# Loveof1ife7/mini-3d-gaussian-splatting

Measured on AMD Instinct MI355X. Metric: rendered Mpix/s fwd+bwd @1080p, 1M Gaussians; PSNR vs ref; 1/2/4/8-GPU scaling, higher is better.
Workload: dtype f32; 1 GPU; C3: 1,000,000 synthetic Gaussians (SURVEY 8d), 1920x1080, 16x16 tiles, render fwd+bwd + Adam step; preset=C3, gaussians=1000000, width=1920, height=1080, parallelism=dp1 (one view per GPU)

## Files before the change

mini-3d-gaussian-splatting_amd/csrc/gs_bin.hip:

```cpp
#include <hip/hip_runtime.h>
#include <stdint.h>

#include "gsplat_mi355x.h"
#include "gs_internal.h"
#include "gs_device.h"

namespace {

#ifndef GS_RANGES_X4
#define GS_RANGES_X4 1
#endif
constexpr int kBinChunk = kBlock * 4;

__device__ __forceinline__ uint2 *sorted_rects(uint32_t *partials, int nb) {
  return reinterpret_cast<uint2 *>(partials + ((5 * nb + 3) & ~3));
}

__global__ __launch_bounds__(kBlock) void k_bin_partials(gs_bin_args a, uint32_t *partials, int nb) {
  __shared__ uint32_t s_tmp3[3][kBlock / kWave];
  const long long base = (long long)blockIdx.x * kBinChunk;
  constexpr int kR = kBinChunk / kBlock;
  uint32_t gi[kR];
  uint2 rc_own[kR];
#pragma unroll
  for (int i = 0; i < kR; ++i) {
    const long long k = base + i * kBlock + threadIdx.x;
    const long long kc = k < a.n ? k : a.n - 1;
    gi[i] = a.sorted_ids[kc];
    rc_own[i] = reinterpret_cast<const uint2 *>(a.rects)[kc];
  }
  uint32_t sum = 0, nvis = 0;
  uint2 rc_d[kR];
  uint32_t vis_o[kR];
#pragma unroll
  for (int i = 0; i < kR; ++i) {
    const long long k = base + i * kBlock + threadIdx.x;
    rc_d[i] = reinterpret_cast<const uint2 *>(a.rects)[gi[i]];
    vis_o[i] = a.vis[k < a.n ? k : a.n - 1];
  }
#pragma unroll
  for (int i = 0; i < kR; ++i) {
    const long long k = base + i * kBlock + threadIdx.x;
    if (k < a.n) {
      sum += rect_touches((int)(rc_d[i].x & 0xFFFFu), (int)(rc_d[i].x >> 16), (int)(rc_d[i].y & 0xFFFFu),
                          (int)(rc_d[i].y >> 16));
      nvis += vis_o[i] ? 1u : 0u;
    }
  }
  uint32_t cnt[kR];
#pragma unroll
  for (int i = 0; i < kR; ++i) {
    const long long g = base + i * kBlock + threadIdx.x;
    cnt[i] = g < a.n ? rect_touches((int)(rc_own[i].x & 0xFFFFu), (int)(rc_own[i].x >> 16),
                                    (int)(rc_own[i].y & 0xFFFFu), (int)(rc_own[i].y >> 16))
                     : 0u;
  }
  uint3 t3;
  const uint3 e3 = block_exscan3(make_uint3(sum, nvis, cnt[0]), s_tmp3, &t3);
  if (threadIdx.x == 0) {
    partials[blockIdx.x] = t3.x;
    partials[nb + blockIdx.x] = t3.y;
  }
  uint2 *srect = sorted_rects(partials, nb);
#pragma unroll
  for (int i = 0; i < kR; ++i) {
    const long long k = base + i * kBlock + threadIdx.x;
    if (k < a.n) srect[k] = rc_d[i];
  }
  static_assert(kR == 4, "the slot prefix scans assume four rounds per binning block");
  uint3 u3;
  const uint3 f3 = block_exscan3(make_uint3(cnt[1], cnt[2], cnt[3]), s_tmp3, &u3);
  const uint32_t ex[kR] = {e3.z, f3.x, f3.y, f3.z};
  const uint32_t tt[kR] = {t3.z, u3.x, u3.y, u3.z};
  uint32_t carry = 0;
#pragma unroll
  for (int i = 0; i < kR; ++i) {
    const long long g = base + i * kBlock + threadIdx.x;
    if (g < a.n) a.pair_offset[g] = carry + ex[i];
    carry += tt[i];
  }
  if (threadIdx.x == 0) partials[2 * nb + blockIdx.x] = carry;
  constexpr int kPB = kBinChunk / kBlock;
  if (threadIdx.x < kPB) {
    const int pb = blockIdx.x * kPB + threadIdx.x, npb = (a.n + kBlock - 1) / kBlock;
    const bool ok = pb < npb;
    uint32_t mn = ok ? a.key_minmax[2 * pb] : 0xFFFFFFFFu, mx = ok ? a.key_minmax[2 * pb + 1] : 0u;
#pragma unroll
    for (int d = 1; d < kPB; d <<= 1) {
      mn = min(mn, (uint32_t)__shfl_xor((int)mn, d, 64));
      mx = max(mx, (uint32_t)__shfl_xor((int)mx, d, 64));
    }
    if (threadIdx.x == 0) {
      partials[3 * nb + blockIdx.x] = mn;
      partials[4 * nb + blockIdx.x] = mx;
    }
  }
}

__device__ __forceinline__ bool window_held(uint32_t key_base, int key_bits, uint32_t zmin, uint32_t zmax) {
  if (key_bits <= 0 || key_bits >= 32 || zmin > zmax) return true;
  const uint64_t full = (1ull << key_bits) - 1ull;
  const uint64_t lim = key_bits >= 9 ? min(full, 255ull << (key_bits - 8)) : full;
  return zmin >= key_base && (uint64_t)(zmax - key_base) < lim;
}

__global__ __launch_bounds__(kBlock) void k_bin_scan_partials(gs_bin_args a, uint32_t *partials, int nb) {
  uint32_t *const counters = a.counters, *const host_counters = a.host_counters;
  __shared__ uint32_t s_tmp3[3][kBlock / kWave];
  __shared__ uint32_t s_mm[2][kBlock / kWave];
  uint32_t mn = 0xFFFFFFFFu, mx = 0u;
  uint32_t carry = 0, vis = 0, slots = 0;
  auto ld = [&](int i, uint32_t *v) {
    const int ci = i < nb ? i : nb - 1;
    v[0] = partials[ci];
    v[1] = partials[nb + ci];
    v[2] = partials[2 * nb + ci];
    v[3] = partials[3 * nb + ci];
    v[4] = partials[4 * nb + ci];
  };
  uint32_t vn[5];
  ld((int)threadIdx.x, vn);
  for (int c = 0; c < nb; c += kBlock) {
    const int i = c + threadIdx.x;
    const uint32_t v0 = i < nb ? vn[0] : 0u, v1 = i < nb ? vn[1] : 0u, v2 = i < nb ? vn[2] : 0u;
    mn = min(mn, vn[3]);
    mx = max(mx, vn[4]);
    ld(i + kBlock, vn);
    uint3 t3;
    const uint3 e = block_exscan3(make_uint3(v0, v1, v2), s_tmp3, &t3);
    if (i < nb) {
      partials[i] = carry + e.x;
      partials[2 * nb + i] = slots + e.z;
    }
    carry += t3.x;
    vis += t3.y;
    slots += t3.z;
  }
#pragma unroll
  for (int d = 32; d >= 1; d >>= 1) {
    mn = min(mn, (uint32_t)__shfl_xor((int)mn, d, 64));
    mx = max(mx, (uint32_t)__shfl_xor((int)mx, d, 64));
  }
  if ((threadIdx.x & (kWave - 1)) == 0) {
    s_mm[0][threadIdx.x >> 6] = mn;
    s_mm[1][threadIdx.x >> 6] = mx;
  }
  __syncthreads();
  if (threadIdx.x == 0) {
#pragma unroll
    for (int w = 0; w < kBlock / kWave; ++w) {
      mn = min(mn, s_mm[0][w]);
      mx = max(mx, s_mm[1][w]);
    }
    uint32_t status = 0u;
    if ((long long)carry > a.capacity) status |= GS_FRAME_NEED_CAPACITY;
    if (!window_held(a.key_base, a.key_bits, mn, mx)) status |= GS_FRAME_WINDOW_MISS;
    if (vis == 0u) status |= GS_FRAME_EMPTY;
    counters[0] = vis;
    counters[1] = carry;
    counters[2] = mn;
    counters[3] = mx;
    counters[4] = status;
    counters[5] = status ? 0u : carry;
    uint32_t seq = a.host_seq;
    if (a.frame_seq) {
      seq = *a.frame_seq + 1u;
      *a.frame_seq = seq;
    }
    uint32_t sticky = status;
    bool first_fail = status != 0u;
    if (a.step_flags) {
      const uint32_t old = atomicOr(a.step_flags, status);
      sticky = old | status;
      first_fail = old == 0u && status != 0u;
    }
    if (host_counters) {
      host_counters[0] = vis;
      host_counters[1] = carry;
      host_counters[2] = mn;
      host_counters[3] = mx;
      host_counters[5] = status;
      host_counters[6] = sticky;
      if (first_fail) host_counters[7] = seq;
      __threadfence_system();
      host_counters[4] = seq;
      __threadfence_system();
    }
  }
}

constexpr uint32_t kWaveFillRun = 32;
template <typename Fill>
__device__ __forceinline__ void wave_fill_runs(bool wide, uint32_t lo, uint32_t hi, uint32_t value, Fill fill) {
  unsigned long long m = __ballot(wide);
  if (!m) return;
  const unsigned long long act = __ballot(1);
  const uint32_t lane = threadIdx.x & 63u;
  const uint32_t nact = (uint32_t)__popcll(act), rank = (uint32_t)__popcll(act & ((1ull << lane) - 1ull));
  while (m) {
    const int l = __ffsll(m) - 1;
    m &= m - 1;
    const uint32_t rlo = (uint32_t)__shfl((int)lo, l, 64), rhi = (uint32_t)__shfl((int)hi, l, 64);
    const uint32_t v = (uint32_t)__shfl((int)value, l, 64);
    for (uint32_t o = rlo + rank; o < rhi; o += nact) fill(o, v);
  }
}

constexpr uint32_t kOwnerCap = kBlock * 64;
__global__ __launch_bounds__(kBlock) void k_bin_emit(gs_bin_args a, const uint32_t *partials) {
  __shared__ uint32_t s_off[kBlock + 1];
  __shared__ uint32_t s_g[kBlock];
  __shared__ uint2 s_rect[kBlock];
  __shared__ uint32_t s_tmp[4];
  __shared__ uint32_t s_tmp3[3][kBlock / kWave];
  __shared__ uint8_t s_owner[kOwnerCap];
  const long long base = (long long)blockIdx.x * kBinChunk;
  if (a.device_counts && a.counters[4] != 0u) {
    for (int r = 0; r < kBinChunk / kBlock; ++r) {
      const long long g = base + r * kBlock + threadIdx.x;
      if (g < a.n) reinterpret_cast<uint2 *>(const_cast<uint32_t *>(a.rects))[g] = make_uint2(1u, 1u);
    }
    return;
  }
  const uint32_t T = a.counters[1];
  if ((long long)T > a.capacity) return;
  uint32_t out_base = partials[blockIdx.x];
  constexpr int kR = kBinChunk / kBlock;
  uint32_t gr[kR];
  uint2 rcr[kR];
  uint32_t offr[kR];
  const uint2 *srect = sorted_rects(const_cast<uint32_t *>(partials), (int)gridDim.x);
#pragma unroll
  for (int r = 0; r < kR; ++r) {
    const long long k = base + r * kBlock + threadIdx.x;
    const long long kc = k < a.n ? k : a.n - 1;
    gr[r] = a.sorted_ids[kc];
    rcr[r] = srect[kc];
    offr[r] = a.pair_offset[kc];
  }
  static_assert(kR == 4, "the emission's prefix scans assume four rounds per binning block");
  uint32_t cntr[kR];
#pragma unroll
  for (int r = 0; r < kR; ++r) {
    const long long k = base + r * kBlock + threadIdx.x;
    if (k < a.n) {
      cntr[r] = rect_touches((int)(rcr[r].x & 0xFFFFu), (int)(rcr[r].x >> 16), (int)(rcr[r].y & 0xFFFFu),
                             (int)(rcr[r].y >> 16));
    } else {
      cntr[r] = 0u;
      gr[r] = 0xFFFFFFFFu;
      rcr[r] = make_uint2(1u, 1u);
    }
  }
  uint3 ta;
  uint32_t tb;
  const uint3 ea = block_exscan3(make_uint3(cntr[0], cntr[1], cntr[2]), s_tmp3, &ta);
  const uint32_t eb = block_exscan(cntr[3], s_tmp, &tb);
  const uint32_t exr[kR] = {ea.x, ea.y, ea.z, eb}, totr[kR] = {ta.x, ta.y, ta.z, tb};
#pragma unroll
  for (int r = 0; r < kR; ++r) {
    const uint32_t g = gr[r], cnt = cntr[r], ex = exr[r], tot = totr[r];
    const uint2 rc = rcr[r];
    if (r) __syncthreads();
    s_off[threadIdx.x] = ex;
    s_g[threadIdx.x] = g;
    s_rect[threadIdx.x] = rc;
    if (threadIdx.x == 0) s_off[kBlock] = tot;
    for (uint32_t wb = 0; wb < tot; wb += kOwnerCap) {
      if (wb) __syncthreads();
      const uint32_t lo_c = ex > wb ? ex : wb, hi_c = min(ex + cnt, wb + kOwnerCap);
      const bool wide = hi_c > lo_c + kWaveFillRun;
      if (!wide)
        for (uint32_t o = lo_c; o < hi_c; ++o) s_owner[o - wb] = (uint8_t)threadIdx.x;
      wave_fill_runs(wide, lo_c - wb, hi_c - wb, threadIdx.x, [&](uint32_t o, uint32_t owner) {
        s_owner[o] = (uint8_t)owner;
      });
      __syncthreads();
      const uint32_t wend = min(tot, wb + kOwnerCap);
      for (uint32_t o = wb + threadIdx.x; o < wend; o += kBlock) {
        const int lo = s_owner[o - wb];
        const uint2 rr = s_rect[lo];
        const uint32_t tx0 = rr.x & 0xFFFFu, ty0 = rr.y & 0xFFFFu;
        const uint32_t wt = (rr.x >> 16) - tx0 + 1u;
        const uint32_t loc = o - s_off[lo];
        const uint32_t row = loc / wt;
        const uint32_t key = (ty0 + row) * (uint32_t)a.tiles_x + tx0 + (loc - row * wt);
        a.tile_keys[out_base + o] = key;
        a.pair_gauss[out_base + o] = s_g[lo];
      }
    }
    out_base += tot;
  }
  const uint32_t cbase = partials[2 * gridDim.x + blockIdx.x];
#pragma unroll
  for (int r = 0; r < kR; ++r) {
    const long long g = base + r * kBlock + threadIdx.x;
    if (g < a.n) {
      const uint32_t slot = cbase + offr[r];
      a.pair_offset[g] = slot;
      a.records[(size_t)g * GS_RECORD_FLOATS + 10] = __uint_as_float(slot);
    }
  }
}

__global__ __launch_bounds__(kBlock) void k_tile_ranges4(gs_range_args a) {
  const long long p0 = 4 * ((long long)blockIdx.x * kBlock + threadIdx.x);
  const long long T = live_items(a.num_pairs, a.num_pairs_dev);
  if (p0 > T) return;
  const int lane = threadIdx.x & 63;
  uint4 k = make_uint4(0u, 0u, 0u, 0u);
  if (p0 + 3 < T) {
    k = reinterpret_cast<const uint4 *>(a.sorted_keys)[p0 / 4];
  } else {
    if (p0 < T) k.x = a.sorted_keys[p0];
    if (p0 + 1 < T) k.y = a.sorted_keys[p0 + 1];
    if (p0 + 2 < T) k.z = a.sorted_keys[p0 + 2];
  }
  uint32_t before = (uint32_t)__shfl_up((int)k.w, 1, 64);
  if (lane == 0) before = p0 > 0 ? a.sorted_keys[p0 - 1] : 0u;
  if (a.slot_live) {
    if (p0 + 3 < T)
      reinterpret_cast<uint4 *>(a.slot_live)[p0 / 4] = make_uint4(0u, 0u, 0u, 0u);
    else
      for (long long q = p0; q < T; ++q) reinterpret_cast<uint32_t *>(a.slot_live)[q] = 0u;
  }
  const uint32_t kk[4] = {k.x, k.y, k.z, k.w};
#pragma unroll
  for (int i = 0; i < 4; ++i) {
    const long long p = p0 + i;
    const bool in = p <= T;
    const long long prev = !in ? 0 : (p > 0 ? (long long)(i ? kk[i - 1] : before) : -1);
    const long long cur = !in ? 0 : (p < T ? (long long)kk[i] : (long long)a.num_tiles);
    const bool edge = in && cur != prev;
    if (edge && prev >= 0) a.ranges[2 * prev + 1] = (uint32_t)p;
    if (edge && cur < a.num_tiles) a.ranges[2 * cur] = (uint32_t)p;
    const uint32_t t0 = (uint32_t)(prev + 1), t1 = edge ? (uint32_t)cur : t0;
    const bool wide = edge && t1 > t0 + kWaveFillRun;
    if (edge && !wide)
      for (uint32_t t = t0; t < t1; ++t) a.ranges[2 * t] = a.ranges[2 * t + 1] = (uint32_t)p;
    wave_fill_runs(wide, t0, t1, (uint32_t)p, [&](uint32_t t, uint32_t q) { a.ranges[2 * t] = a.ranges[2 * t + 1] = q; });
  }
}

__global__ __launch_bounds__(kBlock) void k_tile_ranges(gs_range_args a) {
  const long long p = (long long)blockIdx.x * kBlock + threadIdx.x;
  a.num_pairs = live_items(a.num_pairs, a.num_pairs_dev);
  if (p > a.num_pairs) return;
  if (a.slot_live && p < a.num_pairs) {
    if (a.cells == 4)
      reinterpret_cast<uint32_t *>(a.slot_live)[p] = 0u;
    else if (a.cells == 1)
      a.slot_live[p] = 0;
    else
      for (int c = 0; c < a.cells; ++c) a.slot_live[p * a.cells + c] = 0;
  }
  const long long prev = p > 0 ? (long long)a.sorted_keys[p - 1] : -1;
  const long long cur = p < a.num_pairs ? (long long)a.sorted_keys[p] : (long long)a.num_tiles;
  const bool edge = cur != prev;
  if (edge && prev >= 0) a.ranges[2 * prev + 1] = (uint32_t)p;
  if (edge && cur < a.num_tiles) a.ranges[2 * cur] = (uint32_t)p;
  const uint32_t t0 = (uint32_t)(prev + 1), t1 = edge ? (uint32_t)cur : t0;
  const bool wide = t1 > t0 + kWaveFillRun;
  if (!wide)
    for (uint32_t t = t0; t < t1; ++t) a.ranges[2 * t] = a.ranges[2 * t + 1] = (uint32_t)p;
  wave_fill_runs(wide, t0, t1, (uint32_t)p, [&](uint32_t t, uint32_t q) { a.ranges[2 * t] = a.ranges[2 * t + 1] = q; });
}

}

extern "C" {

size_t gs_bin_workspace_bytes(int32_t n) {
  const size_t nb = n > 0 ? div_up(n, kBinChunk) : 1;
  return sizeof(uint32_t) * ((5 * nb + 3) & ~(size_t)3) + sizeof(uint32_t) * 2 * (size_t)(n > 0 ? n : 0) + 256;
}

gs_status gs_bin_count(const gs_bin_args *a, gs_stream_t stream) {
  if (!a || !a->counters) return gs_internal_fail(GS_ERR_INVALID_ARG, "%s: null args", "gs_bin_count");
  if (a->n <= 0) return GS_OK;
  if (!a->sorted_ids || !a->rects || !a->vis || !a->pair_offset || !a->workspace || !a->key_minmax ||
      a->workspace_bytes < gs_bin_workspace_bytes(a->n))
    return gs_internal_fail(GS_ERR_INVALID_ARG, "%s: null buffer or workspace too small", "gs_bin_count");
  hipStream_t s = (hipStream_t)stream;
  const int nb = (int)div_up(a->n, kBinChunk);
  uint32_t *partials = (uint32_t *)a->workspace;
  k_bin_partials<<<nb, kBlock, 0, s>>>(*a, partials, nb);
  k_bin_scan_partials<<<1, kBlock, 0, s>>>(*a, partials, nb);
  return gs_internal_check_launch("gs_bin_count");
}

gs_status gs_bin_emit(const gs_bin_args *a, gs_stream_t stream) {
  if (!a) return gs_internal_fail(GS_ERR_INVALID_ARG, "%s: null args", "gs_bin_emit");
  if (a->n <= 0) return GS_OK;
  if (!a->sorted_ids || !a->rects || !a->counters || !a->workspace || !a->tile_keys || !a->pair_gauss ||
      !a->pair_offset || !a->records)
    return gs_internal_fail(GS_ERR_INVALID_ARG, "%s: null buffer", "gs_bin_emit");
  if (a->workspace_bytes < gs_bin_workspace_bytes(a->n))
    return gs_internal_fail(GS_ERR_INVALID_ARG, "%s: workspace too small", "gs_bin_emit");
  if (a->capacity < 0) return gs_internal_fail(GS_ERR_INVALID_ARG, "%s: negative capacity", "gs_bin_emit");
  hipStream_t s = (hipStream_t)stream;
  const int nb = (int)div_up(a->n, kBinChunk);
  k_bin_emit<<<nb, kBlock, 0, s>>>(*a, (const uint32_t *)a->workspace);
  return gs_internal_check_launch("gs_bin_emit");
}

gs_status gs_tile_ranges(const gs_range_args *a, gs_stream_t stream) {
  if (!a || !a->ranges) return gs_internal_fail(GS_ERR_INVALID_ARG, "%s: null args", "gs_tile_ranges");
  hipStream_t s = (hipStream_t)stream;
  if (a->num_pairs < 0 || a->num_tiles < 0) return gs_internal_fail(GS_ERR_INVALID_ARG, "%s: negative size", "gs_tile_ranges");
  if (a->num_tiles == 0) return GS_OK;
  if (a->num_pairs > 0 && !a->sorted_keys) return gs_internal_fail(GS_ERR_INVALID_ARG, "%s: null buffer", "gs_tile_ranges");
  if (a->slot_live && (a->cells < 1 || (a->cells == 4 && (reinterpret_cast<uintptr_t>(a->slot_live) & 3u))))
    return gs_internal_fail(GS_ERR_INVALID_ARG, "%s: slot_live needs cells >= 1 (4-B aligned at 4 cells)", "gs_tile_ranges");
  if (GS_RANGES_X4 && (!a->slot_live || a->cells == 4) && (reinterpret_cast<uintptr_t>(a->sorted_keys) & 15u) == 0 &&
      (reinterpret_cast<uintptr_t>(a->slot_live) & 15u) == 0)
    k_tile_ranges4<<<div_up(a->num_pairs / 4 + 1, kBlock), kBlock, 0, s>>>(*a);
  else
    k_tile_ranges<<<div_up(a->num_pairs + 1, kBlock), kBlock, 0, s>>>(*a);
  return gs_internal_check_launch("gs_tile_ranges");
}

}
```

mini-3d-gaussian-splatting_amd/csrc/gs_internal.h:

```cpp
#pragma once
#include "gsplat_mi355x.h"

__attribute__((visibility("hidden"))) gs_status gs_internal_fail(gs_status s, const char *fmt, const char *what);
__attribute__((visibility("hidden"))) gs_status gs_internal_check_launch(const char *what);

__attribute__((visibility("hidden"))) gs_status gs_internal_radix_sort_pairs(
    uint32_t *keys, uint32_t *vals, uint32_t *keys_alt, uint32_t *vals_alt, int32_t n, int32_t begin_bit,
    int32_t end_bit, int32_t vals_are_iota, void *workspace, size_t workspace_bytes, int32_t *result_in_alt,
    const uint32_t *n_dev, gs_stream_t stream);
__attribute__((visibility("hidden"))) int32_t gs_internal_small_sort_max(void);
__attribute__((visibility("hidden"))) gs_status gs_internal_small_sort(const uint32_t *keys, const uint32_t *vals,
                                                                      uint32_t *keys_out, uint32_t *vals_out,
                                                                      int32_t n, int32_t bits, const uint32_t *n_dev,
                                                                      gs_stream_t stream);
```

mini-3d-gaussian-splatting_amd/csrc/gs_render.hip:

```cpp
#include <hip/hip_runtime.h>
#include <sched.h>
#include <stdint.h>
#include <string.h>

#include <stdio.h>

#include <chrono>

#include "gs_internal.h"
#include "gsplat_mi355x.h"

namespace {

size_t al256(size_t x) { return (x + 255) & ~(size_t)255; }

struct FrameLayout {
  size_t records, rects, keys, vals, key_minmax, counters, sort_ws, bin_ws, pair_offset, ranges, pix_flags,
      cell_neval, grad_sums, total;
};

FrameLayout frame_layout(int32_t n, int32_t W, int32_t H, int32_t tiles, int32_t cells) {
  FrameLayout L;
  const size_t un = (size_t)(n > 0 ? n : 0), hw = (size_t)W * (size_t)H;
  size_t o = 0;
  auto take = [&](size_t bytes) {
    const size_t at = o;
    o += al256(bytes);
    return at;
  };
  L.records = take(un * GS_RECORD_FLOATS * 4);
  L.rects = take(un * 8);
  L.keys = take(un * 8);
  L.vals = take(un * 8);
  L.key_minmax = take(8 * ((un + 255) / 256 + 1));
  L.counters = take(4 * GS_NUM_COUNTERS);
  L.sort_ws = take(gs_radix_sort_workspace_bytes(n > 0 ? n : 1));
  L.bin_ws = take(gs_bin_workspace_bytes(n > 0 ? n : 1));
  L.pair_offset = take(un * 4);
  L.ranges = take((size_t)tiles * 8);
  L.pix_flags = take(hw);
  L.cell_neval = take((size_t)tiles * (size_t)(cells > 0 ? cells : 0) * 4);
  L.grad_sums = take(un * GS_PAIR_GRAD_FLOATS * 4);
  L.total = o;
  return L;
}

struct TileLayout {
  size_t tk[2], tv[2], sort_ws, live, flags, total;
  size_t live_words;
};

TileLayout tile_layout(int64_t cap, int32_t tiles, int32_t live_cells, int32_t flag_groups) {
  TileLayout L;
  const size_t uc = (size_t)(cap > 0 ? cap : 0);
  size_t o = 0;
  auto take = [&](size_t bytes) {
    const size_t at = o;
    o += al256(bytes);
    return at;
  };
  L.tk[0] = take(uc * 4);
  L.tk[1] = take(uc * 4);
  L.tv[0] = take(uc * 4);
  L.tv[1] = take(uc * 4);
  L.sort_ws = take(gs_radix_sort_workspace_bytes((int32_t)(cap > 0 ? cap : 1)));
  L.live_words = live_cells > 0 ? gs_blend_live_words((int32_t)uc, tiles) : 0;
  L.live = take((size_t)(live_cells > 0 ? live_cells : 0) * L.live_words * 8);
  L.flags = take(uc * (size_t)(flag_groups > 0 ? flag_groups : 0));
  L.total = o;
  return L;
}

int32_t div_up_i(int32_t a, int32_t b) { return (a + b - 1) / b; }

bool fb_ok(const gs_frame_buffers &fb, int32_t n, int32_t W, int32_t H, int32_t tiles, int32_t cells,
           size_t *need_frame) {
  const FrameLayout F = frame_layout(n, W, H, tiles, cells);
  *need_frame = F.total;
  return fb.frame_ws && fb.frame_ws_bytes >= F.total;
}

bool window_holds(uint32_t key_base, int32_t key_bits, uint32_t zmin, uint32_t zmax) {
  if (key_bits >= 32 || zmin > zmax) return true;
  const uint64_t full = (1ull << key_bits) - 1ull;
  const uint64_t lim = key_bits >= 9 ? (full < (255ull << (key_bits - 8)) ? full : (255ull << (key_bits - 8))) : full;
  return zmin >= key_base && (uint64_t)(zmax - key_base) < lim;
}

thread_local char g_event_err[256];
hipError_t record_event(hipEvent_t ev, gs_stream_t stream) {
  hipStream_t s = (hipStream_t)stream;
  hipStreamCaptureStatus cs = hipStreamCaptureStatusNone;
  hipGraph_t graph = nullptr;
  const hipGraphNode_t *deps = nullptr;
  size_t ndeps = 0;
  hipError_t e = hipStreamGetCaptureInfo_v2(s, &cs, nullptr, &graph, &deps, &ndeps);
  if (e != hipSuccess) {
    snprintf(g_event_err, sizeof(g_event_err), "%%s: hipStreamGetCaptureInfo_v2: %s", hipGetErrorString(e));
    return e;
  }
  if (cs != hipStreamCaptureStatusActive) {
    e = hipEventRecord(ev, s);
    if (e != hipSuccess) snprintf(g_event_err, sizeof(g_event_err), "%%s: hipEventRecord: %s", hipGetErrorString(e));
    return e;
  }
  hipGraphNode_t node = nullptr;
  e = hipGraphAddEventRecordNode(&node, graph, deps, ndeps, ev);
  if (e == hipSuccess) e = hipStreamUpdateCaptureDependencies(s, &node, 1, hipStreamSetCaptureDependencies);
  if (e != hipSuccess) snprintf(g_event_err, sizeof(g_event_err), "%%s: event record node: %s", hipGetErrorString(e));
  return e;
}

}

extern "C" {

size_t gs_frame_workspace_bytes(int32_t n, int32_t width, int32_t height, int32_t tile_size) {
  if (n < 0 || width <= 0 || height <= 0 || tile_size < 1) return 0;
  const int32_t tiles = div_up_i(width, tile_size) * div_up_i(height, tile_size);
  return frame_layout(n, width, height, tiles, gs_tile_quads(tile_size)).total;
}

size_t gs_tile_workspace_bytes(int64_t capacity, int32_t num_tiles, int32_t live_cells, int32_t flag_groups) {
  if (capacity < 0 || capacity > 0x7fffffffLL || num_tiles < 0 || live_cells < 0 || flag_groups < 0) return 0;
  return tile_layout(capacity, num_tiles, live_cells, flag_groups).total;
}

gs_status gs_render_forward(gs_render_fwd_args *a, gs_stream_t stream) {
  static const char *what = "gs_render_forward";
  if (!a) return gs_internal_fail(GS_ERR_INVALID_ARG, "%s: null args", what);
  if (!(a->filter.variance >= 0.f) || !__builtin_isfinite(a->filter.variance))
    return gs_internal_fail(GS_ERR_INVALID_ARG, "%s: filter.variance must be finite and >= 0", what);
  const int32_t n = a->g.n, W = a->cam.image_width, H = a->cam.image_height, L = a->cam.tile_size;
  if (n < 0 || W <= 0 || H <= 0 || L < 1) return gs_internal_fail(GS_ERR_INVALID_ARG, "%s: bad sizes", what);
  const int32_t tiles_x = div_up_i(W, L), tiles_y = div_up_i(H, L), tiles = tiles_x * tiles_y;
  const int32_t cells = gs_tile_quads(L);
  size_t need = 0;
  if (!fb_ok(a->fb, n, W, H, tiles, cells, &need))
    return gs_internal_fail(GS_ERR_INVALID_ARG, "%s: frame workspace missing or below gs_frame_workspace_bytes", what);
  const bool dev = a->device_counts != 0;
  if (dev && (a->fb.capacity <= 0 || a->resume))
    return gs_internal_fail(GS_ERR_INVALID_ARG, "%s: device_counts needs a tile workspace (capacity > 0), no resume",
                            what);
  if (dev && a->fb.flag_groups > 0 && a->fb.flag_groups < cells)
    return gs_internal_fail(GS_ERR_UNSUPPORTED, "%s: device_counts renders tiles of one backward batch only", what);
  if (!dev && (!a->host_counters_dev || !a->host_counters_host))
    return gs_internal_fail(GS_ERR_INVALID_ARG, "%s: the pinned counter buffer (device and host address) is required",
                            what);
  const FrameLayout F = frame_layout(n, W, H, tiles, cells);
  char *fw = reinterpret_cast<char *>(a->fb.frame_ws);
  float *records = reinterpret_cast<float *>(fw + F.records);
  uint32_t *rects = reinterpret_cast<uint32_t *>(fw + F.rects);
  uint32_t *keys = reinterpret_cast<uint32_t *>(fw + F.keys), *vals = reinterpret_cast<uint32_t *>(fw + F.vals);
  uint32_t *key_minmax = reinterpret_cast<uint32_t *>(fw + F.key_minmax);
  uint32_t *counters = reinterpret_cast<uint32_t *>(fw + F.counters);
  uint32_t *pair_offset = reinterpret_cast<uint32_t *>(fw + F.pair_offset);
  uint32_t *ranges = reinterpret_cast<uint32_t *>(fw + F.ranges);
  gs_status st;
  const size_t un = (size_t)n;
  gs_bin_args ba;
  memset(&ba, 0, sizeof(ba));
  ba.n = n;
  ba.tiles_x = tiles_x;
  ba.tiles_y = tiles_y;
  ba.rects = rects;
  ba.vis = a->vis;
  ba.counters = counters;
  ba.key_minmax = key_minmax;
  ba.workspace = fw + F.bin_ws;
  ba.workspace_bytes = gs_bin_workspace_bytes(n > 0 ? n : 1);
  ba.pair_offset = pair_offset;
  ba.records = records;
  ba.key_base = a->key_base;
  ba.key_bits = a->key_bits;
  ba.step_flags = a->step_flags;
  ba.frame_seq = a->frame_seq;
  ba.device_counts = dev ? 1 : 0;
  if (!a->resume) {
    a->M = a->T = 0;
    a->depth_min_bits = 0xFFFFFFFFu;
    a->depth_max_bits = 0u;
    gs_project_args pa;
    memset(&pa, 0, sizeof(pa));
    pa.cam = a->cam;
    pa.g = a->g;
    pa.means2d = a->means2d;
    pa.conics = a->conics;
    pa.radii = a->radii;
    pa.vis = a->vis;
    pa.records = records;
    pa.rects = rects;
    pa.depth_keys = keys;
    pa.key_base = a->key_base;
    pa.key_bits = a->key_bits;
    pa.key_minmax = key_minmax;
    pa.filter = a->filter;
    if ((st = gs_project_forward(&pa, stream))) return st;
    if (n == 0) return GS_OK;
    int32_t alt = 0;
    if (n <= gs_internal_small_sort_max()) {
      st = gs_internal_small_sort(keys, nullptr, keys + un, vals + un, n, a->key_bits, nullptr, stream);
      alt = 1;
    } else if (a->depth_sort_msd && a->key_bits >= 9 && a->key_bits <= 31)
      st = gs_depth_sort_msd(keys, vals, keys + un, vals + un, n, a->key_bits, fw + F.sort_ws,
                             gs_radix_sort_workspace_bytes(n), key_minmax + 1, &alt, stream);
    else
      st = gs_radix_sort_pairs(keys, vals, keys + un, vals + un, n, 0, a->key_bits, 1, fw + F.sort_ws,
                               gs_radix_sort_workspace_bytes(n), &alt, stream);
    if (st) return st;
    a->depth_alt = alt;
  }
  ba.sorted_ids = vals + (a->depth_alt ? un : 0);
  if (n == 0) return GS_OK;
  const TileLayout T0 = tile_layout(a->fb.capacity, tiles, a->fb.live_cells, a->fb.flag_groups);
  if (a->fb.capacity > 0 && (!a->fb.tile_ws || a->fb.tile_ws_bytes < T0.total))
    return gs_internal_fail(GS_ERR_INVALID_ARG, "%s: tile workspace below gs_tile_workspace_bytes(capacity, ...)", what);
  char *tw = reinterpret_cast<char *>(a->fb.tile_ws);
  ba.capacity = a->fb.capacity;
  ba.tile_keys = a->fb.capacity > 0 ? reinterpret_cast<uint32_t *>(tw + T0.tk[0]) : nullptr;
  ba.pair_gauss = a->fb.capacity > 0 ? reinterpret_cast<uint32_t *>(tw + T0.tv[0]) : nullptr;
  const int32_t bits = tiles > 1 ? 32 - __builtin_clz((uint32_t)(tiles - 1)) : 1;
  if (dev) {
    ba.host_counters = a->host_counters_dev;
    ba.host_seq = a->host_seq;
    if ((st = gs_bin_count(&ba, stream))) return st;
    if ((st = gs_bin_emit(&ba, stream))) return st;
    a->M = a->T = -1;
  } else if (!a->resume) {
    ba.host_counters = a->host_counters_dev;
    ba.host_seq = a->host_seq;
    volatile uint32_t *hc = a->host_counters_host;
    hc[4] = 0u;
    if ((st = gs_bin_count(&ba, stream))) return st;
    if (a->fb.capacity > 0 && (st = gs_bin_emit(&ba, stream))) return st;
    const auto t0 = std::chrono::steady_clock::now();
    for (uint32_t i = 1; hc[4] != a->host_seq; ++i) {
      if ((i & 1023u) == 0) {
        if (std::chrono::steady_clock::now() - t0 > std::chrono::seconds(a->poll_timeout_ms > 0 ? 0 : 10) +
                                                        std::chrono::milliseconds(a->poll_timeout_ms)) {
          if (hipStreamSynchronize((hipStream_t)stream) != hipSuccess)
            return gs_internal_fail(GS_ERR_LAUNCH, "%s: hipStreamSynchronize failed while waiting for the counters",
                                    what);
          if (hc[4] != a->host_seq)
            return gs_internal_fail(GS_ERR_LAUNCH, "%s: the frame's counters never reached the host", what);
          break;
        }
        sched_yield();
      }
    }
    __atomic_thread_fence(__ATOMIC_ACQUIRE);
    a->M = (int32_t)hc[0];
    a->T = (int32_t)hc[1];
    a->depth_min_bits = hc[2];
    a->depth_max_bits = hc[3];
    if (!window_holds(a->key_base, a->key_bits, a->depth_min_bits, a->depth_max_bits))
      return GS_RETRY_FULL_KEYS;
    if (a->M == 0) return GS_OK;
    if ((int64_t)a->T > a->fb.capacity) return GS_NEED_CAPACITY;
  } else {
    if ((int64_t)a->T > a->fb.capacity)
      return gs_internal_fail(GS_ERR_INVALID_ARG, "%s: resume needs a capacity of at least T", what);
    if ((st = gs_bin_emit(&ba, stream))) return st;
  }
  const int32_t T = dev ? (int32_t)a->fb.capacity : a->T;
  const uint32_t *t_dev = dev ? counters + 5 : nullptr;
  int32_t talt = 0;
  uint32_t *tk = reinterpret_cast<uint32_t *>(tw + T0.tk[0]), *tk1 = reinterpret_cast<uint32_t *>(tw + T0.tk[1]);
  uint32_t *tv = reinterpret_cast<uint32_t *>(tw + T0.tv[0]), *tv1 = reinterpret_cast<uint32_t *>(tw + T0.tv[1]);
  if (T <= gs_internal_small_sort_max()) {
    if ((st = gs_internal_small_sort(tk, tv, tk1, tv1, T, bits, t_dev, stream))) return st;
    talt = 1;
  } else if ((st = gs_internal_radix_sort_pairs(tk, tv, tk1, tv1, T, 0, bits, 0, tw + T0.sort_ws,
                                                gs_radix_sort_workspace_bytes((int32_t)a->fb.capacity), &talt, t_dev,
                                                stream))) {
    return st;
  }
  a->tile_alt = talt;
  gs_range_args ra;
  memset(&ra, 0, sizeof(ra));
  ra.num_pairs = T;
  ra.num_tiles = tiles;
  ra.sorted_keys = talt ? tk1 : tk;
  ra.ranges = ranges;
  ra.slot_live = (a->zero_slot_flags && a->fb.flag_groups > 0) ? reinterpret_cast<uint8_t *>(tw + T0.flags) : nullptr;
  ra.cells = a->fb.flag_groups;
  ra.num_pairs_dev = t_dev;
  if ((st = gs_tile_ranges(&ra, stream))) return st;
  gs_blend_fwd_args fa;
  memset(&fa, 0, sizeof(fa));
  fa.cam = a->cam;
  fa.tiles_x = tiles_x;
  fa.tiles_y = tiles_y;
  fa.ranges = ranges;
  fa.sorted_gauss = talt ? tv1 : tv;
  fa.records = records;
  fa.image = a->image;
  fa.alpha = a->alpha;
  fa.depth = a->depth;
  fa.pix_flags = reinterpret_cast<uint8_t *>(fw + F.pix_flags);
  fa.cell_neval = reinterpret_cast<uint32_t *>(fw + F.cell_neval);
  fa.pix_neval = a->pix_neval;
  fa.live_bits = a->fb.live_cells > 0 ? reinterpret_cast<uint64_t *>(tw + T0.live) : nullptr;
  fa.live_words = (int64_t)T0.live_words;
  fa.pair_counts = a->pair_counts;
  fa.num_pairs = T;
  return gs_blend_forward(&fa, stream);
}

gs_status gs_render_backward(gs_render_bwd_args *a, gs_stream_t stream) {
  static const char *what = "gs_render_backward";
  if (!a) return gs_internal_fail(GS_ERR_INVALID_ARG, "%s: null args", what);
  if (!(a->filter.variance >= 0.f) || !__builtin_isfinite(a->filter.variance))
    return gs_internal_fail(GS_ERR_INVALID_ARG, "%s: filter.variance must be finite and >= 0", what);
  const int32_t n = a->g.n, W = a->cam.image_width, H = a->cam.image_height, L = a->cam.tile_size;
  if (n < 0 || W <= 0 || H <= 0 || L < 1) return gs_internal_fail(GS_ERR_INVALID_ARG, "%s: bad sizes", what);
  const int32_t tiles_x = div_up_i(W, L), tiles_y = div_up_i(H, L), tiles = tiles_x * tiles_y;
  const int32_t cells = gs_tile_quads(L), G = a->fb.flag_groups;
  size_t need = 0;
  if (!fb_ok(a->fb, n, W, H, tiles, cells, &need))
    return gs_internal_fail(GS_ERR_INVALID_ARG, "%s: frame workspace missing or below gs_frame_workspace_bytes", what);
  const FrameLayout F = frame_layout(n, W, H, tiles, cells);
  char *fw = reinterpret_cast<char *>(a->fb.frame_ws);
  float *grad_sums = reinterpret_cast<float *>(fw + F.grad_sums);
  a->grad_sums = grad_sums;
  gs_status st;
  const bool dev = a->device_counts != 0;
  if (dev && (a->fb.capacity <= 0 || G < cells))
    return gs_internal_fail(GS_ERR_INVALID_ARG, "%s: device_counts needs the forward's capacity and one batch", what);
  const bool pixel_grads = (dev || (a->M > 0 && a->T > 0)) && a->g_image;
  const int32_t T = dev ? (int32_t)a->fb.capacity : a->T;
  if (pixel_grads) {
    if (!a->pair_grads || G < 1) return gs_internal_fail(GS_ERR_INVALID_ARG, "%s: pair_grads / flag_groups", what);
    if (!a->image || !a->alpha || !a->depth)
      return gs_internal_fail(GS_ERR_INVALID_ARG, "%s: the forward's image / alpha / depth are required", what);
    const TileLayout T0 = tile_layout(a->fb.capacity, tiles, a->fb.live_cells, G);
    char *tw = reinterpret_cast<char *>(a->fb.tile_ws);
    if (!tw || a->fb.tile_ws_bytes < T0.total)
      return gs_internal_fail(GS_ERR_INVALID_ARG, "%s: tile workspace below gs_tile_workspace_bytes", what);
    uint8_t *flags = reinterpret_cast<uint8_t *>(tw + T0.flags);
    gs_blend_bwd_args b;
    memset(&b, 0, sizeof(b));
    b.cam = a->cam;
    b.tiles_x = tiles_x;
    b.tiles_y = tiles_y;
    b.ranges = reinterpret_cast<const uint32_t *>(fw + F.ranges);
    b.sorted_gauss = reinterpret_cast<const uint32_t *>(tw + (a->tile_alt ? T0.tv[1] : T0.tv[0]));
    b.records = reinterpret_cast<const float *>(fw + F.records);
    b.image = a->image;
    b.alpha = a->alpha;
    b.depth = a->depth;
    b.pix_flags = reinterpret_cast<const uint8_t *>(fw + F.pix_flags);
    b.cell_neval = reinterpret_cast<const uint32_t *>(fw + F.cell_neval);
    b.g_image = a->g_image;
    b.g_alpha = a->g_alpha;
    b.g_depth = a->g_depth;
    b.live_bits = a->fb.live_cells > 0 ? reinterpret_cast<const uint64_t *>(tw + T0.live) : nullptr;
    b.live_words = (int64_t)T0.live_words;
    b.pair_grads = a->pair_grads;
    b.slot_live = flags;
    b.num_pairs = T;
    gs_project_bwd_args ga;
    memset(&ga, 0, sizeof(ga));
    ga.g.n = n;
    ga.vis = a->vis;
    ga.rects = reinterpret_cast<const uint32_t *>(fw + F.rects);
    ga.pair_offset = reinterpret_cast<const uint32_t *>(fw + F.pair_offset);
    ga.pair_grads = a->pair_grads;
    ga.slot_live = flags;
    ga.grad_sums = grad_sums;
    hipEvent_t ev0 = (hipEvent_t)a->blend_events[0], ev1 = (hipEvent_t)a->blend_events[1];
    if (ev0 && record_event(ev0, stream) != hipSuccess)
      return gs_internal_fail(GS_ERR_LAUNCH, g_event_err, what);
    const int32_t one = gs_partial_groups(L);
    if (G >= one || G >= cells) {
      b.cell_begin = 0;
      b.cell_count = 0;
      ga.partial_groups = G;
      if (!a->flags_zeroed && hipMemsetAsync(flags, 0, (size_t)T * (size_t)G, (hipStream_t)stream) != hipSuccess)
        return gs_internal_fail(GS_ERR_LAUNCH, "%s: slot flag memset failed", what);
      if ((st = gs_blend_backward(&b, stream))) return st;
      if (ev1 && record_event(ev1, stream) != hipSuccess)
        return gs_internal_fail(GS_ERR_LAUNCH, g_event_err, what);
      if ((st = gs_gather_partials(&ga, 0, stream))) return st;
    } else {
      for (int32_t c0 = 0, bi = 0; c0 < cells; c0 += G, ++bi) {
        b.cell_begin = c0;
        b.cell_count = cells - c0 < G ? cells - c0 : G;
        ga.partial_groups = b.cell_count;
        if ((bi || !a->flags_zeroed) &&
            hipMemsetAsync(flags, 0, (size_t)T * (size_t)G, (hipStream_t)stream) != hipSuccess)
          return gs_internal_fail(GS_ERR_LAUNCH, "%s: slot flag memset failed", what);
        if ((st = gs_blend_backward(&b, stream))) return st;
        if ((st = gs_gather_partials(&ga, bi ? 1 : 0, stream))) return st;
      }
      if (ev1 && record_event(ev1, stream) != hipSuccess)
        return gs_internal_fail(GS_ERR_LAUNCH, g_event_err, what);
    }
  }
  if (!a->project) return GS_OK;
  gs_project_bwd_args pb;
  memset(&pb, 0, sizeof(pb));
  pb.cam = a->cam;
  pb.g = a->g;
  pb.means2d = a->means2d;
  pb.conics = a->conics;
  pb.vis = a->vis;
  pb.rects = reinterpret_cast<const uint32_t *>(fw + F.rects);
  pb.pair_offset = reinterpret_cast<const uint32_t *>(fw + F.pair_offset);
  pb.g_means2d = a->g_means2d;
  pb.g_conics = a->g_conics;
  pb.d_xyz = a->d_xyz;
  pb.d_cov3d = a->d_cov3d;
  pb.d_scaling = a->d_scaling;
  pb.d_rotation = a->d_rotation;
  pb.d_color_logits = a->d_color_logits;
  pb.d_opacity = a->d_opacity;
  pb.d_sh_rest = a->d_sh_rest;
  pb.grad_sums = pixel_grads ? grad_sums : nullptr;
  pb.filter = a->filter;
  if (a->fused_adam) return gs_project_backward_adam(&pb, a->fused_adam, stream);
  return gs_project_backward(&pb, stream);
}

void gs_frame_offsets(int32_t n, int32_t width, int32_t height, int32_t tile_size, size_t out[14]) {
  if (!out) return;
  const int32_t tiles = (width > 0 && height > 0 && tile_size > 0)
                            ? div_up_i(width, tile_size) * div_up_i(height, tile_size) : 0;
  const FrameLayout F = frame_layout(n, width > 0 ? width : 0, height > 0 ? height : 0, tiles,
                                     tile_size > 0 ? gs_tile_quads(tile_size) : 0);
  const size_t v[14] = {F.records, F.rects,  F.keys,    F.vals,      F.key_minmax, F.counters,  F.sort_ws,
                        F.bin_ws,  F.pair_offset, F.ranges, F.pix_flags, F.cell_neval, F.grad_sums, F.total};
  memcpy(out, v, sizeof(v));
}

void gs_tile_offsets(int64_t capacity, int32_t num_tiles, int32_t live_cells, int32_t flag_groups, size_t out[9]) {
  if (!out) return;
  const TileLayout T = tile_layout(capacity, num_tiles, live_cells, flag_groups);
  const size_t v[9] = {T.tk[0], T.tk[1], T.tv[0], T.tv[1], T.sort_ws, T.live, T.flags, T.total, T.live_words};
  memcpy(out, v, sizeof(v));
}

}
```

Measured before the change: 1854 Mpix/s.

## Fold the single-block partials scan into every emit block

Removes the one-block k_bin_scan_partials launch. Each k_bin_emit block now reduces all per-block partials itself to get the total, its own prefix offsets and the depth min/max, and block 0 writes the frame counters. This cuts one serialized, low-occupancy kernel and a launch gap from the binning chain. In exchange every emit block redundantly reads the full partials array, which holds about 1000 entries for 1M Gaussians. The resume path also reruns the partials kernel, and an env var can turn the fused path off.

```diff
diff --git a/mini-3d-gaussian-splatting_amd/csrc/gs_bin.hip b/mini-3d-gaussian-splatting_amd/csrc/gs_bin.hip
--- a/mini-3d-gaussian-splatting_amd/csrc/gs_bin.hip
+++ b/mini-3d-gaussian-splatting_amd/csrc/gs_bin.hip
@@ -104,8 +104,51 @@
   return zmin >= key_base && (uint64_t)(zmax - key_base) < lim;
 }
 
+__device__ __forceinline__ uint32_t frame_status(const gs_bin_args &a, uint32_t vis, uint32_t carry, uint32_t mn,
+                                                 uint32_t mx) {
+  uint32_t status = 0u;
+  if ((long long)carry > a.capacity) status |= GS_FRAME_NEED_CAPACITY;
+  if (!window_held(a.key_base, a.key_bits, mn, mx)) status |= GS_FRAME_WINDOW_MISS;
+  if (vis == 0u) status |= GS_FRAME_EMPTY;
+  return status;
+}
+
+__device__ __forceinline__ void write_frame_counters(const gs_bin_args &a, uint32_t vis, uint32_t carry, uint32_t mn,
+                                                     uint32_t mx, uint32_t status) {
+  uint32_t *const counters = a.counters, *const host_counters = a.host_counters;
+  counters[0] = vis;
+  counters[1] = carry;
+  counters[2] = mn;
+  counters[3] = mx;
+  counters[4] = status;
+  counters[5] = status ? 0u : carry;
+  uint32_t seq = a.host_seq;
+  if (a.frame_seq) {
+    seq = *a.frame_seq + 1u;
+    *a.frame_seq = seq;
+  }
+  uint32_t sticky = status;
+  bool first_fail = status != 0u;
+  if (a.step_flags) {
+    const uint32_t old = atomicOr(a.step_flags, status);
+    sticky = old | status;
+    first_fail = old == 0u && status != 0u;
+  }
+  if (host_counters) {
+    host_counters[0] = vis;
+    host_counters[1] = carry;
+    host_counters[2] = mn;
+    host_counters[3] = mx;
+    host_counters[5] = status;
+    host_counters[6] = sticky;
+    if (first_fail) host_counters[7] = seq;
+    __threadfence_system();
+    host_counters[4] = seq;
+    __threadfence_system();
+  }
+}
+
 __global__ __launch_bounds__(kBlock) void k_bin_scan_partials(gs_bin_args a, uint32_t *partials, int nb) {
-  uint32_t *const counters = a.counters, *const host_counters = a.host_counters;
   __shared__ uint32_t s_tmp3[3][kBlock / kWave];
   __shared__ uint32_t s_mm[2][kBlock / kWave];
   uint32_t mn = 0xFFFFFFFFu, mx = 0u;
@@ -152,40 +195,7 @@
       mn = min(mn, s_mm[0][w]);
       mx = max(mx, s_mm[1][w]);
     }
-    uint32_t status = 0u;
-    if ((long long)carry > a.capacity) status |= GS_FRAME_NEED_CAPACITY;
-    if (!window_held(a.key_base, a.key_bits, mn, mx)) status |= GS_FRAME_WINDOW_MISS;
-    if (vis == 0u) status |= GS_FRAME_EMPTY;
-    counters[0] = vis;
-    counters[1] = carry;
-    counters[2] = mn;
-    counters[3] = mx;
-    counters[4] = status;
-    counters[5] = status ? 0u : carry;
-    uint32_t seq = a.host_seq;
-    if (a.frame_seq) {
-      seq = *a.frame_seq + 1u;
-      *a.frame_seq = seq;
-    }
-    uint32_t sticky = status;
-    bool first_fail = status != 0u;
-    if (a.step_flags) {
-      const uint32_t old = atomicOr(a.step_flags, status);
-      sticky = old | status;
-      first_fail = old == 0u && status != 0u;
-    }
-    if (host_counters) {
-      host_counters[0] = vis;
-      host_counters[1] = carry;
-      host_counters[2] = mn;
-      host_counters[3] = mx;
-      host_counters[5] = status;
-      host_counters[6] = sticky;
-      if (first_fail) host_counters[7] = seq;
-      __threadfence_system();
-      host_counters[4] = seq;
-      __threadfence_system();
-    }
+    write_frame_counters(a, vis, carry, mn, mx, frame_status(a, vis, carry, mn, mx));
   }
 }
 
@@ -207,6 +217,7 @@
 }
 
 constexpr uint32_t kOwnerCap = kBlock * 64;
+template <bool kFused>
 __global__ __launch_bounds__(kBlock) void k_bin_emit(gs_bin_args a, const uint32_t *partials) {
   __shared__ uint32_t s_off[kBlock + 1];
   __shared__ uint32_t s_g[kBlock];
@@ -215,29 +226,84 @@
   __shared__ uint32_t s_tmp3[3][kBlock / kWave];
   __shared__ uint8_t s_owner[kOwnerCap];
   const long long base = (long long)blockIdx.x * kBinChunk;
-  if (a.device_counts && a.counters[4] != 0u) {
-    for (int r = 0; r < kBinChunk / kBlock; ++r) {
-      const long long g = base + r * kBlock + threadIdx.x;
-      if (g < a.n) reinterpret_cast<uint2 *>(const_cast<uint32_t *>(a.rects))[g] = make_uint2(1u, 1u);
-    }
-    return;
-  }
-  const uint32_t T = a.counters[1];
-  if ((long long)T > a.capacity) return;
-  uint32_t out_base = partials[blockIdx.x];
   constexpr int kR = kBinChunk / kBlock;
   uint32_t gr[kR];
   uint2 rcr[kR];
   uint32_t offr[kR];
   const uint2 *srect = sorted_rects(const_cast<uint32_t *>(partials), (int)gridDim.x);
-#pragma unroll
-  for (int r = 0; r < kR; ++r) {
-    const long long k = base + r * kBlock + threadIdx.x;
-    const long long kc = k < a.n ? k : a.n - 1;
-    gr[r] = a.sorted_ids[kc];
-    rcr[r] = srect[kc];
-    offr[r] = a.pair_offset[kc];
-  }
+  auto load_rounds = [&]() __attribute__((always_inline)) {
+#pragma unroll
+    for (int r = 0; r < kR; ++r) {
+      const long long k = base + r * kBlock + threadIdx.x;
+      const long long kc = k < a.n ? k : a.n - 1;
+      gr[r] = a.sorted_ids[kc];
+      rcr[r] = srect[kc];
+      offr[r] = a.pair_offset[kc];
+    }
+  };
+  uint32_t f_out_base = 0u, f_cbase = 0u, f_status = 0u, f_T = 0u;
+  if constexpr (kFused) {
+    load_rounds();
+    __shared__ uint32_t s_red[6][kBlock / kWave];
+    const int nb = (int)gridDim.x, b = (int)blockIdx.x;
+    uint32_t sT = 0u, sM = 0u, pT = 0u, pS = 0u, mn = 0xFFFFFFFFu, mx = 0u;
+#pragma unroll 4
+    for (int c = 0; c < nb; c += kBlock) {
+      const int i = c + (int)threadIdx.x, ci = i < nb ? i : nb - 1;
+      const uint32_t v0 = partials[ci], v1 = partials[nb + ci], v2 = partials[2 * nb + ci];
+      mn = min(mn, partials[3 * nb + ci]);
+      mx = max(mx, partials[4 * nb + ci]);
+      sT += i < nb ? v0 : 0u;
+      sM += i < nb ? v1 : 0u;
+      pT += i < b ? v0 : 0u;
+      pS += i < b ? v2 : 0u;
+    }
+#pragma unroll
+    for (int d = 32; d >= 1; d >>= 1) {
+      sT += (uint32_t)__shfl_xor((int)sT, d, 64);
+      sM += (uint32_t)__shfl_xor((int)sM, d, 64);
+      pT += (uint32_t)__shfl_xor((int)pT, d, 64);
+      pS += (uint32_t)__shfl_xor((int)pS, d, 64);
+      mn = min(mn, (uint32_t)__shfl_xor((int)mn, d, 64));
+      mx = max(mx, (uint32_t)__shfl_xor((int)mx, d, 64));
+    }
+    if ((threadIdx.x & (kWave - 1)) == 0) {
+      const int w = threadIdx.x >> 6;
+      s_red[0][w] = sT;
+      s_red[1][w] = sM;
+      s_red[2][w] = pT;
+      s_red[3][w] = pS;
+      s_red[4][w] = mn;
+      s_red[5][w] = mx;
+    }
+    __syncthreads();
+    sT = sM = pT = pS = 0u;
+#pragma unroll
+    for (int w = 0; w < kBlock / kWave; ++w) {
+      sT += s_red[0][w];
+      sM += s_red[1][w];
+      pT += s_red[2][w];
+      pS += s_red[3][w];
+      mn = min(mn, s_red[4][w]);
+      mx = max(mx, s_red[5][w]);
+    }
+    f_T = sT;
+    f_out_base = pT;
+    f_cbase = pS;
+    f_status = frame_status(a, sM, f_T, mn, mx);
+    if (b == 0 && threadIdx.x == 0) write_frame_counters(a, sM, f_T, mn, mx, f_status);
+  }
+  if (a.device_counts && (kFused ? f_status : a.counters[4]) != 0u) {
+    for (int r = 0; r < kBinChunk / kBlock; ++r) {
+      const long long g = base + r * kBlock + threadIdx.x;
+      if (g < a.n) reinterpret_cast<uint2 *>(const_cast<uint32_t *>(a.rects))[g] = make_uint2(1u, 1u);
+    }
+    return;
+  }
+  const uint32_t T = kFused ? f_T : a.counters[1];
+  if ((long long)T > a.capacity) return;
+  uint32_t out_base = kFused ? f_out_base : partials[blockIdx.x];
+  if constexpr (!kFused) load_rounds();
   static_assert(kR == 4, "the emission's prefix scans assume four rounds per binning block");
   uint32_t cntr[kR];
 #pragma unroll
@@ -291,7 +357,7 @@
     }
     out_base += tot;
   }
-  const uint32_t cbase = partials[2 * gridDim.x + blockIdx.x];
+  const uint32_t cbase = kFused ? f_cbase : partials[2 * gridDim.x + blockIdx.x];
 #pragma unroll
   for (int r = 0; r < kR; ++r) {
     const long long g = base + r * kBlock + threadIdx.x;
@@ -366,16 +432,7 @@
   wave_fill_runs(wide, t0, t1, (uint32_t)p, [&](uint32_t t, uint32_t q) { a.ranges[2 * t] = a.ranges[2 * t + 1] = q; });
 }
 
-}
-
-extern "C" {
-
-size_t gs_bin_workspace_bytes(int32_t n) {
-  const size_t nb = n > 0 ? div_up(n, kBinChunk) : 1;
-  return sizeof(uint32_t) * ((5 * nb + 3) & ~(size_t)3) + sizeof(uint32_t) * 2 * (size_t)(n > 0 ? n : 0) + 256;
-}
-
-gs_status gs_bin_count(const gs_bin_args *a, gs_stream_t stream) {
+gs_status bin_count(const gs_bin_args *a, bool scan, gs_stream_t stream) {
   if (!a || !a->counters) return gs_internal_fail(GS_ERR_INVALID_ARG, "%s: null args", "gs_bin_count");
   if (a->n <= 0) return GS_OK;
   if (!a->sorted_ids || !a->rects || !a->vis || !a->pair_offset || !a->workspace || !a->key_minmax ||
@@ -385,11 +442,11 @@
   const int nb = (int)div_up(a->n, kBinChunk);
   uint32_t *partials = (uint32_t *)a->workspace;
   k_bin_partials<<<nb, kBlock, 0, s>>>(*a, partials, nb);
-  k_bin_scan_partials<<<1, kBlock, 0, s>>>(*a, partials, nb);
+  if (scan) k_bin_scan_partials<<<1, kBlock, 0, s>>>(*a, partials, nb);
   return gs_internal_check_launch("gs_bin_count");
 }
 
-gs_status gs_bin_emit(const gs_bin_args *a, gs_stream_t stream) {
+gs_status bin_emit(const gs_bin_args *a, bool fused, gs_stream_t stream) {
   if (!a) return gs_internal_fail(GS_ERR_INVALID_ARG, "%s: null args", "gs_bin_emit");
   if (a->n <= 0) return GS_OK;
   if (!a->sorted_ids || !a->rects || !a->counters || !a->workspace || !a->tile_keys || !a->pair_gauss ||
@@ -400,9 +457,30 @@
   if (a->capacity < 0) return gs_internal_fail(GS_ERR_INVALID_ARG, "%s: negative capacity", "gs_bin_emit");
   hipStream_t s = (hipStream_t)stream;
   const int nb = (int)div_up(a->n, kBinChunk);
-  k_bin_emit<<<nb, kBlock, 0, s>>>(*a, (const uint32_t *)a->workspace);
+  if (fused)
+    k_bin_emit<true><<<nb, kBlock, 0, s>>>(*a, (const uint32_t *)a->workspace);
+  else
+    k_bin_emit<false><<<nb, kBlock, 0, s>>>(*a, (const uint32_t *)a->workspace);
   return gs_internal_check_launch("gs_bin_emit");
 }
+
+}
+
+gs_status gs_internal_bin_partials(const gs_bin_args *a, gs_stream_t stream) { return bin_count(a, false, stream); }
+
+gs_status gs_internal_bin_emit_fused(const gs_bin_args *a, gs_stream_t stream) { return bin_emit(a, true, stream); }
+
+extern "C" {
+
+size_t gs_bin_workspace_bytes(int32_t n) {
+  const size_t nb = n > 0 ? div_up(n, kBinChunk) : 1;
+  return sizeof(uint32_t) * ((5 * nb + 3) & ~(size_t)3) + sizeof(uint32_t) * 2 * (size_t)(n > 0 ? n : 0) + 256;
+}
+
+gs_status gs_bin_count(const gs_bin_args *a, gs_stream_t stream) { return bin_count(a, true, stream); }
+
+gs_status gs_bin_emit(const gs_bin_args *a, gs_stream_t stream) { return bin_emit(a, false, stream); }
+
 
 gs_status gs_tile_ranges(const gs_range_args *a, gs_stream_t stream) {
   if (!a || !a->ranges) return gs_internal_fail(GS_ERR_INVALID_ARG, "%s: null args", "gs_tile_ranges");
diff --git a/mini-3d-gaussian-splatting_amd/csrc/gs_internal.h b/mini-3d-gaussian-splatting_amd/csrc/gs_internal.h
--- a/mini-3d-gaussian-splatting_amd/csrc/gs_internal.h
+++ b/mini-3d-gaussian-splatting_amd/csrc/gs_internal.h
@@ -8,6 +8,9 @@
     uint32_t *keys, uint32_t *vals, uint32_t *keys_alt, uint32_t *vals_alt, int32_t n, int32_t begin_bit,
     int32_t end_bit, int32_t vals_are_iota, void *workspace, size_t workspace_bytes, int32_t *result_in_alt,
     const uint32_t *n_dev, gs_stream_t stream);
+__attribute__((visibility("hidden"))) gs_status gs_internal_bin_partials(const gs_bin_args *a, gs_stream_t stream);
+__attribute__((visibility("hidden"))) gs_status gs_internal_bin_emit_fused(const gs_bin_args *a, gs_stream_t stream);
+
 __attribute__((visibility("hidden"))) int32_t gs_internal_small_sort_max(void);
 __attribute__((visibility("hidden"))) gs_status gs_internal_small_sort(const uint32_t *keys, const uint32_t *vals,
                                                                       uint32_t *keys_out, uint32_t *vals_out,
diff --git a/mini-3d-gaussian-splatting_amd/csrc/gs_render.hip b/mini-3d-gaussian-splatting_amd/csrc/gs_render.hip
--- a/mini-3d-gaussian-splatting_amd/csrc/gs_render.hip
+++ b/mini-3d-gaussian-splatting_amd/csrc/gs_render.hip
@@ -1,6 +1,7 @@
 #include <hip/hip_runtime.h>
 #include <sched.h>
 #include <stdint.h>
+#include <stdlib.h>
 #include <string.h>
 
 #include <stdio.h>
@@ -72,6 +73,11 @@
 }
 
 int32_t div_up_i(int32_t a, int32_t b) { return (a + b - 1) / b; }
+
+bool fused_binning() {
+  const char *e = getenv("GS_FUSED_BINNING");
+  return !(e && e[0] == '0' && e[1] == '\0');
+}
 
 bool fb_ok(const gs_frame_buffers &fb, int32_t n, int32_t W, int32_t H, int32_t tiles, int32_t cells,
            size_t *need_frame) {
@@ -176,6 +182,8 @@
   ba.step_flags = a->step_flags;
   ba.frame_seq = a->frame_seq;
   ba.device_counts = dev ? 1 : 0;
+  const bool fuse_scan = fused_binning();
+  const bool fused = fuse_scan && a->fb.capacity > 0;
   if (!a->resume) {
     a->M = a->T = 0;
     a->depth_min_bits = 0xFFFFFFFFu;
@@ -223,16 +231,26 @@
   if (dev) {
     ba.host_counters = a->host_counters_dev;
     ba.host_seq = a->host_seq;
-    if ((st = gs_bin_count(&ba, stream))) return st;
-    if ((st = gs_bin_emit(&ba, stream))) return st;
+    if (fused) {
+      if ((st = gs_internal_bin_partials(&ba, stream))) return st;
+      if ((st = gs_internal_bin_emit_fused(&ba, stream))) return st;
+    } else {
+      if ((st = gs_bin_count(&ba, stream))) return st;
+      if ((st = gs_bin_emit(&ba, stream))) return st;
+    }
     a->M = a->T = -1;
   } else if (!a->resume) {
     ba.host_counters = a->host_counters_dev;
     ba.host_seq = a->host_seq;
     volatile uint32_t *hc = a->host_counters_host;
     hc[4] = 0u;
-    if ((st = gs_bin_count(&ba, stream))) return st;
-    if (a->fb.capacity > 0 && (st = gs_bin_emit(&ba, stream))) return st;
+    if (fused) {
+      if ((st = gs_internal_bin_partials(&ba, stream))) return st;
+      if ((st = gs_internal_bin_emit_fused(&ba, stream))) return st;
+    } else {
+      if ((st = gs_bin_count(&ba, stream))) return st;
+      if (a->fb.capacity > 0 && (st = gs_bin_emit(&ba, stream))) return st;
+    }
     const auto t0 = std::chrono::steady_clock::now();
     for (uint32_t i = 1; hc[4] != a->host_seq; ++i) {
       if ((i & 1023u) == 0) {
@@ -260,7 +278,12 @@
   } else {
     if ((int64_t)a->T > a->fb.capacity)
       return gs_internal_fail(GS_ERR_INVALID_ARG, "%s: resume needs a capacity of at least T", what);
-    if ((st = gs_bin_emit(&ba, stream))) return st;
+    if (fuse_scan) {
+      if ((st = gs_internal_bin_partials(&ba, stream))) return st;
+      if ((st = gs_internal_bin_emit_fused(&ba, stream))) return st;
+    } else if ((st = gs_bin_emit(&ba, stream))) {
+      return st;
+    }
   }
   const int32_t T = dev ? (int32_t)a->fb.capacity : a->T;
   const uint32_t *t_dev = dev ? counters + 5 : nullptr;
```

Measured after the change: 1858 Mpix/s (median of 3 runs). Within noise of the previous version (+0.2%).
